# mitchelldurbincs/GeneralsReinforcementLearning

Measured on AMD Instinct MI355X. Metric: env steps/sec (whole node), 20x20 4P fog-on; state bit-exact vs the C restatement of the Go engine (the reference's own test vectors pass on both), higher is better.
Workload: dtype int32

## Files before the change

### generalsreinforcementlearning_amd/csrc/gvec_device.hpp

```cpp
#pragma once
#include <hip/hip_runtime.h>
#include <stdint.h>

#include "../../include/generals_vec.h"

extern "C" __device__ int gvec_llvm_writelane(int value, int lane, int vdst_in) __asm("llvm.amdgcn.writelane.i32");

#ifndef GVEC_NT
#define GVEC_NT 14
#endif
#define GVEC_NT_MASK 2
#define GVEC_NT_PLANE 4
#define GVEC_NT_ARMY 8
#ifndef GVEC_SC1
#define GVEC_SC1 1
#endif

#ifndef GVEC_LEAN
#define GVEC_LEAN 7
#endif

#ifndef GVEC_XLANE
#define GVEC_XLANE 28
#endif
#define GVEC_XL_SPREAD 1
#define GVEC_XL_ROW0 2
#define GVEC_XL_ORROWS 4
#define GVEC_XL_ROWLAST 8
#define GVEC_XL_GATHER 16

namespace gvec {

constexpr bool lean_derive_ok(int nslot) { return (GVEC_LEAN & 1) != 0 && 2 * nslot < 64 / (nslot <= 7 ? 4 : 2); }
constexpr bool lean_half_last(int nslot, bool odd) { return (GVEC_LEAN & 2) != 0 && odd && (nslot & 1) != 0; }
constexpr int lean_fold_dwords(int mutable_planes, int fd) { return (GVEC_LEAN & 4) != 0 ? ((mutable_planes * fd + 3) & ~3) - mutable_planes * fd : 0; }
constexpr bool xlane_tight(int maxp, int nslot) { return maxp >= 8 && nslot <= 1; }
constexpr bool xlane_swaps_ok(int maxp, int nslot) { return !(maxp >= 8 && nslot >= 16) && !xlane_tight(maxp, nslot); }
constexpr bool xlane_spread(int maxp, int nslot) { return (GVEC_XLANE & 1) != 0 && xlane_swaps_ok(maxp, nslot); }
constexpr bool xlane_or_rows(int maxp, int nslot) { return (GVEC_XLANE & 4) != 0 && xlane_swaps_ok(maxp, nslot); }
constexpr bool xlane_gather(int maxp, int nslot) { return (GVEC_XLANE & 16) != 0 && !xlane_tight(maxp, nslot); }

typedef uint32_t u32x4 __attribute__((ext_vector_type(4)));

template <typename T>
__device__ __forceinline__ T ld_stream(const T* p) {
  if constexpr ((GVEC_NT & 1) != 0) return __builtin_nontemporal_load(p);
  return *p;
}
__device__ __forceinline__ void st_through(uint32_t* p, uint32_t v) { asm volatile("global_store_dword %0, %1, off sc1 nt" : : "v"(p), "v"(v) : "memory"); }
__device__ __forceinline__ void st_through(uint16_t* p, uint16_t v) {
  asm volatile("global_store_short %0, %1, off sc1 nt" : : "v"(p), "v"((uint32_t)v) : "memory");
}
__device__ __forceinline__ void st_through(float* p, float v) { asm volatile("global_store_dword %0, %1, off sc1 nt" : : "v"(p), "v"(v) : "memory"); }
__device__ __forceinline__ void st_through(u32x4* p, u32x4 v) {
  asm volatile("global_store_dwordx4 %0, %1, off sc1 nt\n\ts_nop 1" : : "v"(p), "v"(v) : "memory");
}
template <int CLASS, typename T>
__device__ __forceinline__ void st_stream(T* p, T v) {
  if constexpr ((GVEC_NT & CLASS) != 0) {
    if constexpr (GVEC_SC1 != 0) st_through(p, v);
    else __builtin_nontemporal_store(v, p);
  } else {
    *p = v;
  }
}

constexpr int HDR_DW = 24;
enum : int {
  H_TURN = 0,
  H_DIMS = 1,
  H_STATUS = 2,
  H_EPISODE = 3,
  H_ARMYCNT = 4,
  H_GIDX = 12,
  H_RECIPW = 20,
  H_CNT_STEPS = 21,
  H_CNT_ABORT = 22,
  H_CNT_DONE = 23
};
constexpr uint32_t HF_DONE = 1u, HF_FOG = 2u, HF_WIDE = 4u;
constexpr uint32_t HF_SETUP = 8u;
constexpr uint32_t HF_SYNC = 16u;
constexpr uint32_t HF_VSMALL = 32u;
constexpr uint32_t HF_LDIFF = 128u;
constexpr uint32_t HF_FEWSPECIAL = 64u;

template <int MAXP>
struct Planes {
  static constexpr int OWN = 0, VIS = MAXP, CHG = 2 * MAXP, VCH = 2 * MAXP + 1, GT1 = 2 * MAXP + 2,
                       GEN = 2 * MAXP + 3, CITY = 2 * MAXP + 4, MTN = 2 * MAXP + 5, VALID = 2 * MAXP + 6, NCOL0 = 2 * MAXP + 7,
                       NCOLL = 2 * MAXP + 8, OK = 2 * MAXP + 9 , LST = 2 * MAXP + 13,
                       COUNT = 3 * MAXP + 13, MUTABLE = 2 * MAXP + 3, SHARED = 13 ;
};

template <int MAXP_, int NSLOT_, bool ODD_>
struct VariantGeom {
  static constexpr int MAXP = MAXP_, NSLOT = NSLOT_;
  static constexpr bool ODD = ODD_;
  static constexpr int FD = 2 * NSLOT - (ODD ? 1 : 0);
  static constexpr int ROW_DW = (Planes<MAXP>::COUNT * FD + 3) / 4 * 4;
  static constexpr int GYM_STAGE_DW = (NSLOT * 64 * 5 + 15) / 16 * 4;
  static_assert(GYM_STAGE_DW >= NSLOT * 64, "the larger user of the gym step kernels' army shadow: the stage serves as both");
};

constexpr uint32_t KF_AGENT = 1u;
constexpr uint32_t KF_EMIT = 2u;
constexpr uint32_t KF_AUTORESET = 4u;
constexpr uint32_t KF_LMVALID = 16u;

struct StepArgs {
  uint32_t* hdr;
  uint32_t* rows;
  uint32_t* army16;
  int32_t* army32;
  const gvec_action* actions;
  gvec_action* actions_out;
  int32_t* err;
  uint32_t* legal;
  const uint32_t* zeros;
  const uint32_t* pool_hdr;
  const uint32_t* pool_rows;
  const uint32_t* pool_army16;
  const int32_t* pool_army32;
// ... 438 lines not shown
```

### generalsreinforcementlearning_amd/csrc/gvec_kernels.hip

```cpp
#include "gvec_dispatch.hpp"
#include "gvec_turn.hpp"

namespace gvec {

template <int MAXP, int NSLOT>
constexpr int step_waves() {
  const int state = Turn<MAXP, NSLOT>::STATE_REGS;
  return waves_for_regs(state + (state + 32 <= 62 ? 32 : 40));
}

template <int MAXP, int NSLOT, bool AGENT, bool ODD>
__global__ __launch_bounds__(64 * WAVES_PER_BLOCK, (step_waves<MAXP, NSLOT>())) void step_kernel(StepArgs A) {
  constexpr int FD = VariantGeom<MAXP, NSLOT, ODD>::FD, ROW_DW = VariantGeom<MAXP, NSLOT, ODD>::ROW_DW;
  __shared__ int32_t army_shadow[WAVES_PER_BLOCK][NSLOT * 64];
  using B = Turn<MAXP, NSLOT>;
  __shared__ uint32_t act_scratch[WAVES_PER_BLOCK][B::ACT_SCRATCH_DW];
  const int wave = block_wave(), lane = lane_id();
  const int env = wave_item();
  if (env >= A.num_envs) return;
  bool force_redeal = false;
  if constexpr (!AGENT) {
    const uint32_t f0 = (uint32_t)uni((int)reinterpret_cast<const uint32_t*>(A.actions)[((size_t)env * A.pstride) * 2 + 1]);
    if (f0 & GVEC_ACT_SKIP_ENV) {
      if (A.err && lane == 0) A.err[env] = 0;
      return;
    }
    force_redeal = (f0 & GVEC_ACT_RESET_ENV) != 0u;
  }
  B b;
  b.larmy = army_shadow[wave];
  b.lscr = act_scratch[wave];
  const ArmyRef army_env = army_ref<NSLOT>(A.army16, A.army32, env);
  load_turn<true, lean_half_last(NSLOT, ODD)>(b, A.hdr + (size_t)env * HDR_DW, A.rows + (size_t)env * ROW_DW, army_env, FD, A.zeros);
  b.small = !(b.hflags & HF_WIDE);
  const bool emit = (A.flags & KF_EMIT) != 0u;
  uint32_t m[B::NR][4];
  uint32_t err = 0u;
  bool types_dirty = false, changed = true;
  const bool can_redeal = (A.flags & KF_AUTORESET) && A.pool_size > 0;
  if (AGENT && A.actions_out && (b.hflags & HF_DONE)) {
    if (lane < A.pstride) reinterpret_cast<uint2*>(A.actions_out)[(size_t)env * A.pstride + lane] = make_uint2(0u, 0u);
  }
  if (can_redeal && ((b.hflags & HF_DONE) || force_redeal)) {
    redeal<MAXP, NSLOT>(b, A, env, FD, ROW_DW);
    types_dirty = true;
  } else if (b.hflags & HF_DONE) {
    err = GVEC_ERR_GAME_OVER;
    changed = false;
  } else {
    typename B::ActVec av;
    if constexpr (AGENT) {
      b.template legal_planes<false>(m);
      uint32_t mine = (GVEC_PROFILE_SKIP & 1) ? 0u : agent_sample<MAXP, NSLOT>(b, m, env_key_of(A.seed_base, (uint32_t)env), A);
      if (GVEC_PROFILE_DUP & 64) { b.opaque(); b.template legal_planes<false>(m); }
      if (GVEC_PROFILE_DUP & 1) {
        b.opaque();
#pragma unroll
        for (int d = 0; d < 4; ++d) asm volatile("" : "+v"(m[0][d]));
        const uint32_t again = agent_sample<MAXP, NSLOT>(b, m, env_key_of(A.seed_base, (uint32_t)env), A);
        asm volatile("" : : "v"(again));
      }
      av = agent_actvec<MAXP, NSLOT>(b, mine, A.invalid_permille > 0);
      if (A.actions_out) {
        uint32_t alo, ahi;
        agent_words<MAXP, NSLOT>(b, mine, alo, ahi);
        if (lane < A.pstride) reinterpret_cast<uint2*>(A.actions_out)[(size_t)env * A.pstride + lane] = make_uint2(alo, ahi);
      }
    } else {
      uint32_t alo = 0u, ahi = 0u;
      if (lane < A.pstride) {
        const uint2 w = reinterpret_cast<const uint2*>(A.actions)[(size_t)env * A.pstride + lane];
        alo = w.x;
        ahi = w.y;
      }
      av = b.prevalidate(alo, ahi);
    }
    bool aborted;
    err = b.turn_step(av, A, aborted);
    if (!(GVEC_PROFILE_SKIP & 32)) b.refresh_gt1();
    if (GVEC_PROFILE_DUP & 32) { b.opaque_v(); b.refresh_gt1(); }
    hdr_set(b, H_CNT_STEPS, hdr_get(b, H_CNT_STEPS) + 1u);
    if (aborted) hdr_set(b, H_CNT_ABORT, hdr_get(b, H_CNT_ABORT) + 1u);
    if (b.hflags & HF_DONE) hdr_set(b, H_CNT_DONE, hdr_get(b, H_CNT_DONE) + 1u);
  }
  store_army<true>(b, army_env);
  settle_lists(b);
  b.store_hdr(A.hdr + (size_t)env * HDR_DW, err);
  if (types_dirty) b.store_planes(A.rows + (size_t)env * ROW_DW, FD, ROW_DW, true);
  else b.store_planes_staged(A.rows + (size_t)env * ROW_DW, FD);
  if (A.err && lane == 0) A.err[env] = (int32_t)err;
  if (!(GVEC_PROFILE_SKIP & 64) && emit && (changed || !(A.flags & KF_LMVALID))) {
    b.template legal_planes<false>(m);
    b.store_masks_staged(m, A.legal + (size_t)env * A.pstride * A.mask_dw, FD, A.pstride);
  }
}

template <int MAXP, int NSLOT>
__global__ __launch_bounds__(64 * WAVES_PER_BLOCK, (rollout_waves<MAXP, NSLOT>())) void rollout_kernel(StepArgs A) {
  __shared__ int32_t army_shadow[WAVES_PER_BLOCK][NSLOT * 64];
  using B = Turn<MAXP, NSLOT>;
  __shared__ uint32_t act_scratch[WAVES_PER_BLOCK][B::ACT_SCRATCH_DW];
  const int wave = block_wave(), lane = lane_id();
  const int env = wave_item();
  if (env >= A.num_envs) return;
  B b;
  b.larmy = army_shadow[wave];
  b.lscr = act_scratch[wave];
  const ArmyRef army_env = army_ref<NSLOT>(A.army16, A.army32, env);
  load_turn(b, A.hdr + (size_t)env * HDR_DW, A.rows + (size_t)env * A.row_dw, army_env, A.fd, A.zeros);
  uint32_t m[B::NR][4];
  uint32_t err = 0u, n_steps = 0u, n_abort = 0u, n_done = 0u;
  const uint32_t ek = env_key_of(A.seed_base, (uint32_t)env);
  const bool can_redeal = (A.flags & KF_AUTORESET) && A.pool_size > 0;
  int k = 0;
  for (;;) {
    b.template legal_planes<false>(m);
// ... 419 lines not shown
```

### generalsreinforcementlearning_amd/csrc/gvec_packed.hpp

```cpp
#pragma once
#include "gvec_device.hpp"

#ifndef GVEC_PROFILE_SKIP
#define GVEC_PROFILE_SKIP 0
#endif
#ifndef GVEC_PROFILE_DUP
#define GVEC_PROFILE_DUP 0
#endif
#ifndef GVEC_ACT_VECTOR
#define GVEC_ACT_VECTOR 1
#endif

namespace gvec {

template <int ROWL>
__device__ __forceinline__ uint32_t row_scan_add(uint32_t v) {
  v += dpp0<0x111>(v);
  v += dpp0<0x112>(v);
  v += dpp0<0x114>(v);
  v += dpp0<0x118>(v);
  if constexpr (ROWL == 32) v += dpp0<0x142, 0xa>(v);
  return v;
}
template <int ROWL>
// ... 141 lines not shown
  }
  __device__ __forceinline__ void decode_hdr_scalar(const uint32_t* hdr_env) {
    typedef const __attribute__((address_space(4))) uint32_t* kptr;
    unpack_hdr(*this, [k = (kptr)hdr_env](int i) { return k[i]; });
  }
  __device__ __forceinline__ void land_scalars() {
    asm volatile("" : "+s"(turn), "+s"(W), "+s"(H), "+s"(P), "+s"(hflags), "+s"(alive), "+s"(recipW));
  }
  __device__ __forceinline__ void load_hdr(const uint32_t* hdr_env) {
    issue_hdr(hdr_env);
    decode_hdr(*this);
  }
  __device__ __forceinline__ void land() {
    asm volatile("" : "+v"(hv));
#pragma unroll
    for (int k = 0; k < NR; ++k) {
      asm volatile("" : "+v"(own[k]));
      asm volatile("" : "+v"(lst[k]));
      asm volatile("" : "+v"(vis[k]));
    }
#pragma unroll
    for (int k = 0; k < NSR; ++k) asm volatile("" : "+v"(shp[k]));
  }
  __device__ __forceinline__ void opaque() {
    opaque_v();
    asm volatile("" : "+s"(turn), "+s"(alive), "+s"(hflags));
  }
  __device__ __forceinline__ void opaque_v() {
    asm volatile("" : "+v"(hv));
#pragma unroll
    for (int s = 0; s < NSLOT; ++s) asm volatile("" : "+v"(army[s]));
#pragma unroll
    for (int k = 0; k < NR; ++k) {
      asm volatile("" : "+v"(own[k]));
      asm volatile("" : "+v"(lst[k]));
      asm volatile("" : "+v"(vis[k]));
    }
    asm volatile("" : "+v"(chg));
    asm volatile("" : "+v"(vch));
    asm volatile("" : "+v"(gt1));
  }
  __device__ __forceinline__ void store_hdr(uint32_t* hdr_env, uint32_t last_err) { pack_hdr<false, GVEC_NT_PLANE>(*this, hdr_env, last_err); }

  template <bool PACK = true>
  __device__ __forceinline__ void load_planes(const uint32_t* rows_env, int fd, const uint32_t* zeros) {
    const bool in = col() < fd;
    const uint32_t* lane_base = rows_env + (row() * fd + col());
    if constexpr (PACK) {
#pragma unroll
      for (int k = 0; k < NR; ++k) {
        own[k] = vis[k] = 0u;
        if (in && (k * PPR + row() < MAXP)) {
          own[k] = ld_stream(lane_base + (PL::OWN + k * PPR) * fd);
          vis[k] = ld_stream(lane_base + (PL::VIS + k * PPR) * fd);
        }
      }
#pragma unroll
      for (int k = 0; k < NSR; ++k) {
        shp[k] = 0u;
        if (in && (k * PPR + row() < NPACKED)) shp[k] = ld_stream(lane_base + (PL::CHG + k * PPR) * fd);
      }
    } else {
#pragma unroll
      for (int k = 0; k < NR; ++k) {
        const uint32_t* gp = (in && (k * PPR + row() < MAXP)) ? lane_base : zeros;
        own[k] = ld_stream(gp + (PL::OWN + k * PPR) * fd);
        vis[k] = ld_stream(gp + (PL::VIS + k * PPR) * fd);
      }
      load_lists(rows_env, fd);
      const uint32_t* gs = in ? rows_env + col() : zeros;
      chg = ld_stream(gs + PL::CHG * fd);
      vch = ld_stream(gs + PL::VCH * fd);
      gt1 = ld_stream(gs + PL::GT1 * fd);
      gen = ld_stream(gs + PL::GEN * fd);
      city = ld_stream(gs + PL::CITY * fd);
      mtn = ld_stream(gs + PL::MTN * fd);
      valid = ld_stream(gs + PL::VALID * fd);
      ncol0 = ld_stream(gs + PL::NCOL0 * fd);
      ncolL = ld_stream(gs + PL::NCOLL * fd);
#pragma unroll
      for (int d = 0; d < 4; ++d) ok[d] = ld_stream(gs + (PL::OK + d) * fd);
    }
  }
  __device__ __forceinline__ void load_lists(const uint32_t* rows_env, int fd) {
#pragma unroll
    for (int k = 0; k < NR; ++k) lst[k] = own[k];
    if (hflags & HF_LDIFF) {
      const uint32_t* lane_base = rows_env + (row() * fd + col());
#pragma unroll
      for (int k = 0; k < NR; ++k) {
        lst[k] = 0u;
        if (col() < fd && (k * PPR + row() < MAXP)) lst[k] = lane_base[(PL::LST + k * PPR) * fd];
      }
    }
  }
  __device__ __forceinline__ void store_lists(uint32_t* rows_env, int fd) const {
    if (!(hflags & HF_LDIFF)) return;
    uint32_t* gp = rows_env + row() * fd + col();
#pragma unroll
    for (int k = 0; k < NR; ++k)
      if (col() < fd && (k * PPR + row() < MAXP)) gp[(PL::LST + k * PPR) * fd] = lst[k];
  }
  __device__ __forceinline__ uint32_t shared_plane(int j) const {
    return row_to_all<ROWL, XL_SPREAD>(shp[j / PPR], j % PPR);
  }
  __device__ __forceinline__ void spread_shared() {
    chg = shared_plane(PL::CHG - PL::CHG);
    vch = shared_plane(PL::VCH - PL::CHG);
    gt1 = shared_plane(PL::GT1 - PL::CHG);
    gen = shared_plane(PL::GEN - PL::CHG);
    city = shared_plane(PL::CITY - PL::CHG);
    mtn = shared_plane(PL::MTN - PL::CHG);
    valid = shared_plane(PL::VALID - PL::CHG);
    ncol0 = shared_plane(PL::NCOL0 - PL::CHG);
    ncolL = shared_plane(PL::NCOLL - PL::CHG);
    if constexpr (DERIVE_OK) {
      derive_targets(*this);
    } else {
#pragma unroll
      for (int d = 0; d < 4; ++d) ok[d] = shared_plane(PL::OK + d - PL::CHG);
    }
  }
  __device__ __forceinline__ void store_planes(uint32_t* rows_env, int fd, int row_dw, bool with_types) const {
    const bool in = col() < fd;
    uint32_t* gp = rows_env + row() * fd + col();
#pragma unroll
    for (int k = 0; k < NR; ++k) {
      if (in && (k * PPR + row() < MAXP)) {
        st_stream<GVEC_NT_PLANE>(gp + (PL::OWN + k * PPR) * fd, own[k]);
        st_stream<GVEC_NT_PLANE>(gp + (PL::VIS + k * PPR) * fd, vis[k]);
      }
    }
    store_lists(rows_env, fd);
    static_assert(PL::VCH == PL::CHG + 1 && PL::GT1 == PL::CHG + 2, "the three mutable shared planes are stored as rows of one register");
#pragma unroll
    for (int k = 0; k * PPR < 3; ++k) {
      const int j = k * PPR + row();
      if (in && j < 3) st_stream<GVEC_NT_PLANE>(gp + (PL::CHG + k * PPR) * fd, j == 0 ? chg : (j == 1 ? vch : gt1));
    }
    const int lane = lane_id();
    if (lane < fd) {
      uint32_t* g = rows_env + lane;
      if (with_types) {
        g[PL::GEN * fd] = gen;
        g[PL::CITY * fd] = city;
        g[PL::MTN * fd] = mtn;
        g[PL::VALID * fd] = valid;
        g[PL::NCOL0 * fd] = ncol0;
        g[PL::NCOLL * fd] = ncolL;
#pragma unroll
        for (int d = 0; d < 4; ++d) g[(PL::OK + d) * fd] = ok[d];
      }
    }
    if (with_types && lane < row_dw - PL::COUNT * fd) rows_env[PL::COUNT * fd + lane] = 0u;
  }
  template <bool HALF_LAST = false>
  __device__ __forceinline__ void load_army_narrow(const ArmyCRef& a) { army_load_narrow<NSLOT, HALF_LAST>(army, a.n); }
  __device__ __forceinline__ void load_army_wide_if_flagged(const ArmyCRef& a) {
    if (hflags & HF_WIDE) army_load_wide<NSLOT>(army, a.w);
  }

  __device__ __forceinline__ void army_to_lds() {
#pragma unroll
    for (int s = 0; s < NSLOT; ++s) larmy[64 * s + lane_id()] = army[s];
    wave_lds_fence();
  }
  __device__ __forceinline__ void army_from_lds() {
    wave_lds_fence();
#pragma unroll
    for (int s = 0; s < NSLOT; ++s) army[s] = larmy[64 * s + lane_id()];
  }
  static __device__ __forceinline__ void larmy_store(int32_t* p, int32_t v) { *p = v; }
  __device__ __forceinline__ int army_get(int t) const { return uni(larmy[t]); }
  __device__ __forceinline__ void army_set(int t, int val) {
    if (lane_id() == 0) larmy[t] = val;
  }

  __device__ __forceinline__ bool bit_at(uint32_t shared_plane, int t) const { return (rdlane(shared_plane, t >> 5) >> (t & 31)) & 1u; }
  __device__ __forceinline__ bool bit_at_p(const uint32_t (&reg)[NR], int p, int t) const {
    uint32_t w = 0u;
#pragma unroll
    for (int k = 0; k < NR; ++k) {
      const uint32_t r = rdlane(reg[k], player_lane<ROWL>(p, t >> 5));
      w = (k == p / PPR) ? r : w;
    }
    return (w >> (t & 31)) & 1u;
  }
  __device__ __forceinline__ uint32_t tile_bit(int t) const { return (col() == (t >> 5)) ? (1u << (t & 31)) : 0u; }

  static constexpr bool XL_GATHER = xlane_gather(MAXP, NSLOT);
  static __device__ __forceinline__ int32_t gather_mask(uint32_t plane, int s, int row_base = 0) { return gather_mask_as<XL_GATHER>(plane, s, row_base); }
  static __device__ __forceinline__ uint32_t gather(uint32_t plane, int s, int row_base = 0) { return gather_as<XL_GATHER>(plane, s, row_base); }
  static __device__ __forceinline__ uint32_t replicate_row0(uint32_t plane) { return row_to_all<ROWL, (GVEC_XLANE & GVEC_XL_ROW0) != 0>(plane, 0); }
  __device__ __forceinline__ int count_shared(uint32_t plane) const {
    return (int)rdlane(row_scan_add<ROWL>((uint32_t)__builtin_popcount(plane)), ROWL - 1);
  }
  static __device__ __forceinline__ bool any_bit(uint32_t plane) { return __builtin_amdgcn_ballot_w64(plane != 0u) != 0ull; }
  __device__ __forceinline__ void refresh_gt1() {
    uint32_t g = 0u;
#pragma unroll
    for (int s = 0; s < NSLOT; ++s) ballot_to_row0(g, __builtin_amdgcn_ballot_w64(army[s] > 1), s);
    gt1 = replicate_row0(g);
  }

  __device__ __forceinline__ void update_fog(bool matched = false) {
    if (!(hflags & HF_FOG)) return;
    bool full, none;
    if ((hflags & HF_VSMALL) && turn > 0 && P <= N / 10) {
      full = false;
      none = !any_bit(vch);
    } else {
      const int nv = count_shared(vch);
      full = turn == 0 || nv > N / 10;
      none = nv == 0;
    }
    if (full) {
#pragma unroll
      for (int k = 0; k < NR; ++k) {
        const uint32_t d = dil3(lst[k]);
        vis[k] = lane_flag(alive, k) ? d : 0u;
      }
      return;
    }
    if (none) return;
    const uint32_t near3 = dil3(vch), clr = ~near3;
    const uint32_t near5 = matched ? 0u : dil3(near3);
#pragma unroll
    for (int k = 0; k < NR; ++k) {
      const uint32_t d = dil3(lst[k]);
      const unsigned long long hit = __builtin_amdgcn_ballot_w64((matched ? (d & near3) : (own[k] & near5)) != 0u);
      const bool relit = row_slice<ROWL>(hit, row()) != 0u && lane_flag(alive, k);
      vis[k] = (vis[k] & clr) | (relit ? d : 0u);
    }
  }

  __device__ __forceinline__ uint32_t multi_sum(const int32_t (&acc)[MAXP]) const {
    static_assert(MAXP == 2 || MAXP == 4 || MAXP == 8, "fold levels are written for 2, 4 or 8 players");
    static_assert(H_ARMYCNT == 4, "the final row_shl assumes header lanes 4..4+MAXP-1");
    const int lane = lane_id();
    uint32_t m[MAXP];
#pragma unroll
    for (int p = 0; p < MAXP; ++p) m[p] = (uint32_t)acc[p];
    {
      const bool hi = (lane & 1) != 0;
#pragma unroll
      for (int i = 0; i < MAXP / 2; ++i) {
        const uint32_t keep = hi ? m[2 * i + 1] : m[2 * i], give = hi ? m[2 * i] : m[2 * i + 1];
        m[i] = keep + dpp0<0xB1>(give);
      }
    }
    if constexpr (MAXP >= 4) {
      const bool hi = (lane & 2) != 0;
#pragma unroll
      for (int i = 0; i < MAXP / 4; ++i) {
        const uint32_t keep = hi ? m[2 * i + 1] : m[2 * i], give = hi ? m[2 * i] : m[2 * i + 1];
        m[i] = keep + dpp0<0x4E>(give);
      }
    }
    if constexpr (MAXP >= 8) {
      const bool hi = (lane & 4) != 0;
      const uint32_t keep = hi ? m[1] : m[0], give = hi ? m[0] : m[1];
      m[0] = keep + dpp0<0x124>(give);
    }
    uint32_t r = m[0];
    if constexpr (MAXP <= 2) r += dpp0<0x112>(r);
    if constexpr (MAXP <= 4) r += dpp0<0x114>(r);
    r += dpp0<0x118>(r);
    constexpr bool VALU = XL_ORROWS;
    const LanePair h = with_partner<16, VALU>(r);
    r = h.a + h.b;
    const LanePair g = with_partner<32, VALU>(r);
    r = g.a + g.b;
    return dpp0<0x100 + 12 - MAXP>(r);
  }

  __device__ __forceinline__ void update_stats(bool end_of_turn = false, bool delta = false) {
    bool full;
    if (end_of_turn && !grow && (hflags & HF_FEWSPECIAL) && turn > 0) {
      if (!any_bit(chg)) return;
      full = false;
    } else {
      const int nc = count_shared(chg);
      if (nc == 0 && turn > 0) return;
      full = turn == 0 || nc > N / 5;
    }
    uint32_t moved = 0u;
#pragma unroll
    for (int k = 0; k < NR; ++k) {
      const uint32_t nl = full ? own[k] : (own[k] & (lst[k] | chg));
      moved |= nl ^ lst[k];
      lst[k] = nl;
    }
    const int lane = lane_id();
    if (delta && !full && prod_uniform) {
      uint32_t add = dpp0<0x114>((lane < MAXP) ? (uint32_t)move_delta : 0u);
      static_assert(H_ARMYCNT == 4 && MAXP <= 8, "row_shr:4 lands lanes 0..MAXP-1 on the ArmyCount lanes");
      if (prod_rate != 0) {
#pragma unroll
        for (int k = 0; k < NR; ++k) {
          const uint32_t sc = row_scan_add<ROWL>((uint32_t)__builtin_popcount(prod_mask & lst[k]));
          const int p = lane - H_ARMYCNT;
          const uint32_t got = row_result<ROWL>(sc, p & (PPR - 1));
          add += (p >= 0 && p < MAXP && p / PPR == k) ? __umul24(got, (uint32_t)prod_rate) : 0u;
        }
      }
      hv += (lane >= H_ARMYCNT && lane < H_ARMYCNT + MAXP) ? add : 0u;
      hflags |= HF_SYNC;
      if (!any_bit(moved)) return;
    } else {
      int32_t acc[MAXP];
#pragma unroll
      for (int p = 0; p < MAXP; ++p) acc[p] = 0;
      if (small) {
#pragma unroll
        for (int s = 0; s < NSLOT; ++s) {
#pragma unroll
          for (int p = 0; p < MAXP; ++p)
            acc[p] = (int32_t)mad24((uint32_t)army[s], gather(lst[p / PPR], s, player_row<ROWL>(p)), (uint32_t)acc[p]);
        }
      } else {
#pragma unroll
        for (int s = 0; s < NSLOT; ++s) {
#pragma unroll
          for (int p = 0; p < MAXP; ++p) acc[p] += army[s] & gather_mask(lst[p / PPR], s, player_row<ROWL>(p));
        }
      }
      const uint32_t tot = multi_sum(acc);
      hv = (lane >= H_ARMYCNT && lane < H_ARMYCNT + MAXP) ? tot : hv;
      hflags |= HF_SYNC;
    }
    {
      const int hl = lane - H_GIDX;
#pragma unroll
      for (int k = 0; k < NR; ++k) {
        const uint32_t g = lst[k] & gen;
        const int32_t v = row_scan_max<ROWL>((g != 0u) ? (32 * col() + 31 - __builtin_clz(g)) : -1);
        const uint32_t got = row_result<ROWL>((uint32_t)v, hl & (PPR - 1));
        hv = (hl >= 0 && hl < MAXP && hl / PPR == k) ? got : hv;
      }
      alive = (uint32_t)(__builtin_amdgcn_ballot_w64(hl >= 0 && hl < MAXP && (int32_t)hv >= 0) >> H_GIDX) & ((1u << MAXP) - 1u);
    }
  }

  __device__ __forceinline__ void production(int pg, int pc, int pn, int interval, uint32_t interval_magic) {
    if ((uint32_t)turn < 0x10000u && (uint32_t)interval < 0x10000u) {
      const uint32_t q = __umulhi((uint32_t)turn, interval_magic);
      int32_t r = turn - (int32_t)(q * (uint32_t)interval);
      r = r < 0 ? r + interval : r;
      grow = r == 0;
    } else {
      grow = (turn % interval) == 0;
    }
    uint32_t listed_alive = 0u;
#pragma unroll
    for (int k = 0; k < NR; ++k) listed_alive |= lane_flag(alive, k) ? lst[k] : 0u;
    listed_alive = or_rows(listed_alive);
    const uint32_t mg = (pg > 0) ? (listed_alive & gen) : 0u;
    const uint32_t mc = (pc > 0) ? (listed_alive & city) : 0u;
    uint32_t mn = 0u;
    if (grow && pn > 0) mn = listed_alive & ~(gen | city | mtn) & valid;
    chg |= mg | mc | mn;
    const int an = (grow && pn > 0) ? pn : pc;
    prod_uniform = pg == pc && pc == an;
    prod_mask = mg | mc | mn;
    prod_rate = pg;
    if (prod_uniform) {
      const uint32_t m = prod_mask;
#pragma unroll
      for (int s = 0; s < NSLOT; ++s) army[s] = (int32_t)mad24(gather(m, s), (uint32_t)pg, (uint32_t)army[s]);
    } else {
#pragma unroll
      for (int s = 0; s < NSLOT; ++s) army[s] += (pg & gather_mask(mg, s)) + (pc & gather_mask(mc, s)) + (pn & gather_mask(mn, s));
    }
  }

  __device__ __forceinline__ void check_game_over() {
    const int na = __builtin_popcount(alive);
    const int most = (P > 1) ? 1 : 0;
    const bool over = na <= most;
    hflags = over ? (hflags | HF_DONE) : (hflags & ~HF_DONE);
  }

  struct ActVec {
    uint32_t meta;
    int ft, tt;
  };
  __device__ __forceinline__ ActVec prevalidate(uint32_t alo, uint32_t ahi) const {
    ActVec v;
    const int fx = (int)(int8_t)(alo & 0xFFu), fy = (int)(int8_t)((alo >> 8) & 0xFFu);
    const int tx = (int)(int8_t)((alo >> 16) & 0xFFu), ty = (int)(int8_t)(alo >> 24);
    const bool inb = fx >= 0 && fx < W && fy >= 0 && fy < H && tx >= 0 && tx < W && ty >= 0 && ty < H;
    const int dx = fx - tx, dy = fy - ty;
    const int md = (dx < 0 ? -dx : dx) + (dy < 0 ? -dy : dy);
    uint32_t code = 0u;
    code = (md != 1) ? GVEC_ERR_NOT_ADJACENT : code;
    code = (md == 0) ? GVEC_ERR_MOVE_TO_SELF : code;
    code = (!inb) ? GVEC_ERR_INVALID_COORDINATES : code;
    v.meta = code | ((ahi & GVEC_ACT_VALID) ? 16u : 0u) | ((ahi & GVEC_ACT_HALF) ? 32u : 0u);
    v.ft = __mul24(fy, W) + fx;
    v.tt = __mul24(ty, W) + tx;
    return v;
  }

  template <int PID>
  __device__ __forceinline__ void apply_action(const ActVec& av, uint32_t& first_err, uint64_t& orders, int& n_orders,
                                               uint32_t& elim_seen) {
    const uint32_t m = rdlane(av.meta, PID);
    if (!(m & 16u)) return;
    if (!((alive >> PID) & 1u)) return;
    uint32_t code = m & 15u;
    int fa = 0, ta = 0, ft = 0, tt = 0;
    if (!code) {
      ft = (int)rdlane((uint32_t)av.ft, PID);
      tt = (int)rdlane((uint32_t)av.tt, PID);
      fa = army_get(ft);
      ta = army_get(tt);
      if (!bit_at_p(own, PID, ft)) code = GVEC_ERR_NOT_OWNED;
      else if (fa <= 1) code = GVEC_ERR_INSUFFICIENT_ARMY;
      else if (bit_at(mtn, tt)) code = GVEC_ERR_TARGET_IS_MOUNTAIN;
    }
    if (code) {
      first_err = first_err ? first_err : code;
      return;
    }
    int n = (m & 32u) ? (fa / 2) : (fa - 1);
    n = (n == 0) ? 1 : n;
    const uint32_t fbit = tile_bit(ft), tbit = tile_bit(tt);
    army_set(ft, fa - n);
    chg |= fbit | tbit;
    if (bit_at_p(own, PID, tt)) {
      army_set(tt, ta + n);
    } else if (n > ta) {
      int prev = -1;
#pragma unroll
      for (int q = 0; q < MAXP; ++q)
// ... 54 lines not shown
    }
    const bool own_ft = ((w_ft >> (ft & 31)) & 1u) != 0u;
    const bool mine_tt = ((owner_bits >> lane) & 1u) != 0u;
    const bool mtn_tt = ((bperm(tcol << 2, mtn) >> (tt & 31)) & 1u) != 0u;
    const bool gen_tt = ((bperm(tcol << 2, gen) >> (tt & 31)) & 1u) != 0u;
    uint32_t dyn = mtn_tt ? GVEC_ERR_TARGET_IS_MOUNTAIN : 0u;
    dyn = (fa <= 1) ? GVEC_ERR_INSUFFICIENT_ARMY : dyn;
    dyn = own_ft ? dyn : GVEC_ERR_NOT_OWNED;
    const uint32_t code = cand ? dyn : scode;
    const bool ok = cand && dyn == 0u;
    {
      const unsigned long long em = __builtin_amdgcn_ballot_w64(active && code != 0u);
      if (em && !first_err) first_err = rdlane(code, (int)__builtin_ctzll(em));
    }
    int32_t n = (m & 32u) ? (fa >> 1) : (fa - 1);
    n = n < 1 ? 1 : n;
    const bool take = !mine_tt && n > ta;
    const bool capture = ok && take;
    const int32_t fight = take ? n - ta : ta - n;
    const int32_t new_ta = mine_tt ? ta + n : fight;
    larmy_store(ok ? &larmy[ft] : reinterpret_cast<int32_t*>(s_dummy), fa - n);
    larmy_store(ok ? &larmy[tt] : reinterpret_cast<int32_t*>(s_dummy), new_ta);
    atomicOr(ok ? &s_chg[fcol] : s_dummy, fbit);
    atomicOr(ok ? &s_chg[tcol] : s_dummy, tbit);
    atomicOr(capture ? &s_cap[tcol] : s_dummy, tbit);
    atomicOr(capture ? &s_own[64 * (lane / PPR) + myrow + tcol] : s_dummy, tbit);
    const int32_t burnt = take ? ta : n;
    const int32_t loss = (ok && !mine_tt) ? burnt : 0;
    atomicAdd((loss != 0 && owner_bits != 0u) ? &s_loss[__builtin_ctz(owner_bits | 0x80000000u) & 7] : s_dummy, (uint32_t)loss);
    wave_lds_fence();
    move_delta = -(loss + (int32_t)s_loss[lane & 7]);
    const uint32_t capbits = s_cap[col()];
    chg |= s_chg[col()];
    vch |= capbits;
#pragma unroll
    for (int k = 0; k < NR; ++k) own[k] = (own[k] & ~capbits) | s_own[64 * k + lane];
    unsigned long long el = __builtin_amdgcn_ballot_w64(capture && gen_tt);
    if (el) el = __builtin_amdgcn_ballot_w64(capture && gen_tt && owner_bits != 0u);
    while (el) {
      const int p = (int)__builtin_ctzll(el);
      el &= el - 1ull;
      const int prev = (int)__builtin_ctz(rdlane(owner_bits, p));
      if (!((elim_seen >> prev) & 1u)) {
        orders |= (uint64_t)((uint32_t)prev | ((uint32_t)p << 4)) << (8 * n_orders);
        n_orders++;
        elim_seen |= 1u << prev;
      }
    }
    return true;
  }

  template <int PID>
  __device__ __forceinline__ void act_chain(const ActVec& av, uint32_t& first_err, uint64_t& orders, int& n_orders,
                                            uint32_t& elim_seen) {
    if constexpr (PID < MAXP) {
      if (PID < P) apply_action<PID>(av, first_err, orders, n_orders, elim_seen);
      act_chain<PID + 1>(av, first_err, orders, n_orders, elim_seen);
    }
  }

  __device__ __forceinline__ void eliminate(uint64_t orders, int n_orders) {
    for (int e = 0; e < n_orders; ++e) {
      const int v = (int)((orders >> (8 * e)) & 15u), nw = (int)((orders >> (8 * e + 4)) & 15u);
      uint32_t tiles = 0u;
#pragma unroll
      for (int k = 0; k < NR; ++k) tiles |= (lane_player(k) == v) ? (lst[k] & own[k]) : 0u;
      tiles = or_rows(tiles);
#pragma unroll
      for (int k = 0; k < NR; ++k) {
        own[k] = (lane_player(k) == v) ? (own[k] & ~tiles) : own[k];
        own[k] = (lane_player(k) == nw) ? (own[k] | tiles) : own[k];
      }
      hdr_set(*this, H_GIDX + v, 0xFFFFFFFFu);
      chg |= tiles;
      vch |= tiles;
      hflags &= ~HF_VSMALL;
      alive &= ~(1u << v);
    }
  }

  __device__ __forceinline__ uint32_t turn_step(uint32_t acts_lo, uint32_t acts_hi, const StepArgs& A, bool& aborted) {
    return turn_step(prevalidate(acts_lo, acts_hi), A, aborted);
  }
  __device__ __forceinline__ uint32_t turn_step(const ActVec& av, const StepArgs& A, bool& aborted) {
    aborted = false;
    turn++;
    const bool matched = lists_match(*this);
    if (!(GVEC_PROFILE_SKIP & 2)) update_fog(matched);
    if (GVEC_PROFILE_DUP & 2) { opaque(); update_fog(matched); }
    chg = 0u;
    vch = 0u;
    hflags |= HF_VSMALL;
    bool delta = matched && (hflags & HF_SYNC) != 0u;
    move_delta = 0;
    uint32_t first_err = 0u, elim_seen = 0u;
    uint64_t orders = 0ull;
    int n_orders = 0;
    const unsigned long long present = __builtin_amdgcn_ballot_w64((av.meta & 16u) != 0u && lane_id() < P);
    if (present && !(GVEC_PROFILE_SKIP & 4)) {
      army_to_lds();
      if (!(GVEC_ACT_VECTOR && lscr && act_vector(av, first_err, orders, n_orders, elim_seen))) {
        act_chain<0>(av, first_err, orders, n_orders, elim_seen);
        delta = false;
      }
      army_from_lds();
    }
    if (n_orders > 0) {
      eliminate(orders, n_orders);
      update_stats();
    }
    if (first_err) {
      if (n_orders == 0) hflags &= ~HF_SYNC;
      aborted = true;
      return first_err;
    }
    if (!(GVEC_PROFILE_SKIP & 8)) production(A.prod_general, A.prod_city, A.prod_normal, A.interval, A.interval_magic);
    if (!(GVEC_PROFILE_SKIP & 16)) update_stats(n_orders == 0, delta && n_orders == 0);
    if (GVEC_PROFILE_DUP & 16) { opaque_v(); update_stats(n_orders == 0, false); }
    check_game_over();
    return 0u;
  }

  __device__ __forceinline__ void initial_setup() {
    turn = 0;
    chg = 0u;
    vch = 0u;
#pragma unroll
    for (int k = 0; k < NR; ++k) vis[k] = 0u;
    hflags = (hflags & ~HF_DONE) | HF_VSMALL;
    update_stats();
    update_fog();
    check_game_over();
  }

  template <bool SERIALIZER = false>
  __device__ __forceinline__ void legal_planes(uint32_t (&m)[NR][4]) const {
#pragma unroll
    for (int k = 0; k < NR; ++k) {
      const uint32_t s = SERIALIZER ? (own[k] & gt1) : (lst[k] & own[k] & gt1);
      const uint32_t src = (SERIALIZER || lane_flag(alive, k)) ? s : 0u;
      m[k][0] = src & ok[0];
      m[k][1] = src & (SERIALIZER ? ok[2] : ok[1]);
      m[k][2] = src & (SERIALIZER ? ok[3] : ok[2]);
      m[k][3] = src & (SERIALIZER ? ok[1] : ok[3]);
    }
  }
  __device__ __forceinline__ void store_masks(const uint32_t (&m)[NR][4], uint32_t* legal_env, int fd, int pstride) const {
    const bool in = col() < fd;
#pragma unroll
    for (int k = 0; k < NR; ++k) {
      const int p = lane_player(k);
      if (in && p < pstride && p < MAXP) {
        uint32_t* g = legal_env + (size_t)p * (4 * fd) + col();
#pragma unroll
        for (int d = 0; d < 4; ++d) st_stream<GVEC_NT_MASK>(g + d * fd, m[k][d]);
      }
    }
  }
  template <int CLASS>
  __device__ __forceinline__ void flush_stage(uint32_t* dst, int dwords) const {
    const u32x4* s4 = reinterpret_cast<const u32x4*>(larmy);
    u32x4* g4 = reinterpret_cast<u32x4*>(dst);
    const int chunks = dwords >> 2;
    for (int i = lane_id(); i < chunks; i += 64) {
      st_stream<CLASS>(g4 + i, s4[i]);
    }
    const int tail = dwords & 3, l = lane_id();
    if (l < tail) st_stream<CLASS>(dst + 4 * chunks + l, reinterpret_cast<const uint32_t*>(larmy)[4 * chunks + l]);
  }
  __device__ __forceinline__ void store_planes_staged(uint32_t* rows_env, int fd) const {
    uint32_t* stage = reinterpret_cast<uint32_t*>(larmy);
    const bool in = col() < fd;
    uint32_t* g = stage + row() * fd + col();
    wave_lds_fence();
#pragma unroll
    for (int k = 0; k < NR; ++k) {
      if (in && (k * PPR + row() < MAXP)) {
        g[(PL::OWN + k * PPR) * fd] = own[k];
        g[(PL::VIS + k * PPR) * fd] = vis[k];
      }
    }
#pragma unroll
    for (int k = 0; k * PPR < 3; ++k) {
      const int j = k * PPR + row();
      if (in && j < 3) g[(PL::CHG + k * PPR) * fd] = j == 0 ? chg : (j == 1 ? vch : gt1);
    }
    const int gap = lean_fold_dwords(PL::MUTABLE, fd);
    if (in && row() == 0) {
      if (col() < gap) g[PL::GEN * fd] = gen;
      if (fd + col() < gap) g[PL::CITY * fd] = city;
      if (2 * fd + col() < gap) g[PL::MTN * fd] = mtn;
    }
    wave_lds_fence();
    flush_stage<GVEC_NT_PLANE>(rows_env, PL::MUTABLE * fd + gap);
    store_lists(rows_env, fd);
  }
  __device__ __forceinline__ void store_army_narrow_staged(uint32_t* n) const {
    uint32_t* stage = reinterpret_cast<uint32_t*>(larmy);
    const int lane = lane_id();
    wave_lds_fence();
#pragma unroll
// ... 30 lines not shown
```

### generalsreinforcementlearning_amd/csrc/gvec_turn.hpp

```cpp
#pragma once
#include "gvec_launch.hpp"
#include "gvec_packed.hpp"

namespace gvec {

template <int MAXP, int NSLOT>
using Turn = PBoard<MAXP, NSLOT>;

template <int MAXP, int NSLOT>
__device__ __forceinline__ uint32_t agent_sample(const Turn<MAXP, NSLOT>& b, const uint32_t (&m)[Turn<MAXP, NSLOT>::NR][4], uint32_t ek,
                                                 const StepArgs& A) {
  using T = Turn<MAXP, NSLOT>;
  constexpr int NR = T::NR, PPR = T::PPR, ROWL = T::ROWL;
  const int lane = lane_id();
  const uint32_t sbase = ek + (uint32_t)b.turn * 0x9E3779B1u + 0x165667B1u;
  uint32_t mine = 0u;
#pragma unroll
  for (int k = 0; k < NR; ++k) {
    const uint32_t player = (uint32_t)T::lane_player(k);
    const uint32_t h1 = amix(mad24(player, 0x4A7C15u, sbase));
    const uint32_t h2 = amix(h1 ^ 0x68E31DA4u);
    const uint32_t hi16 = h2 >> 16;
    const bool act = b.lane_flag(b.alive, k) && !((h1 & 0xFFFFu) < A.agent_noop);
    const bool half = (h1 >> 16) < A.agent_half;
    const bool inv = A.invalid_permille > 0 && (__umul24(h2 & 0xFFFFu, 1000u) >> 16) < (uint32_t)A.invalid_permille;
    const uint32_t c0 = (uint32_t)__builtin_popcount(m[k][0]), c1 = c0 + (uint32_t)__builtin_popcount(m[k][1]);
    const uint32_t c2 = c1 + (uint32_t)__builtin_popcount(m[k][2]), cnt = c2 + (uint32_t)__builtin_popcount(m[k][3]);
    const uint32_t sc = row_scan_add<ROWL>(cnt);
    const uint32_t total = row_last<ROWL>(sc);
    const uint32_t kk = __umul24(hi16, total) >> 16;
    const uint32_t below = sc - cnt;
    const bool sel = kk >= below && kk < sc;
    const uint32_t r = kk - below;
    const uint32_t d = (r >= c0 ? 1u : 0u) + (r >= c1 ? 1u : 0u) + (r >= c2 ? 1u : 0u);
    const uint32_t base = (d == 0u) ? 0u : (d == 1u) ? c0 : (d == 2u) ? c1 : c2;
    const uint32_t w = (d == 0u) ? m[k][0] : (d == 1u) ? m[k][1] : (d == 2u) ? m[k][2] : m[k][3];
    const uint32_t t_sel = 32u * (uint32_t)T::col() + kth_set_bit(w, r - base);
    const uint32_t pick = row_scan_or<ROWL>(sel ? (t_sel | (d << 10) | 0x8000u) : 0u);
    const uint32_t unchecked = (__umul24(hi16, (uint32_t)b.N) >> 16) | (((h1 >> 8) & 3u) << 10) | 0x8000u;
    const uint32_t fin = inv ? unchecked : pick;
    const bool go = act && (fin & 0x8000u) != 0u;
    const uint32_t out = (fin & 0xFFFu) | (go ? 0x1000u : 0u) | (half ? 0x2000u : 0u);
    const uint32_t got = row_result<ROWL>(out, lane % PPR);
    mine = (lane / PPR == k) ? got : mine;
  }
  return mine;
}

template <int MAXP, int NSLOT>
__device__ __forceinline__ void agent_words(const Turn<MAXP, NSLOT>& b, uint32_t mine, uint32_t& alo, uint32_t& ahi) {
  const bool act = lane_id() < MAXP && (mine & 0x1000u) != 0u;
  const int t = (int)(mine & 0x3FFu), d = (int)((mine >> 10) & 3u);
  const int y = (int)(__umul24((uint32_t)t, (uint32_t)b.recipW) >> 16), x = t - (int)__umul24((uint32_t)y, (uint32_t)b.W);
  const int dx = (d == 1) - (d == 3), dy = (d == 2) - (d == 0);
  const uint32_t lo = ((uint32_t)x & 0xFFu) | (((uint32_t)y & 0xFFu) << 8) | (((uint32_t)(x + dx) & 0xFFu) << 16) |
                      (((uint32_t)(y + dy) & 0xFFu) << 24);
  alo = act ? lo : 0u;
  ahi = act ? (GVEC_ACT_VALID | ((mine & 0x2000u) ? GVEC_ACT_HALF : 0u)) : 0u;
}

template <int MAXP, int NSLOT>
__device__ __forceinline__ typename Turn<MAXP, NSLOT>::ActVec agent_actvec(const Turn<MAXP, NSLOT>& b, uint32_t mine, bool may_be_unchecked) {
  typename Turn<MAXP, NSLOT>::ActVec v;
  const bool act = lane_id() < MAXP && (mine & 0x1000u) != 0u;
  const int t = (int)(mine & 0x3FFu), d = (int)((mine >> 10) & 3u);
  uint32_t code = 0u;
  if (may_be_unchecked) {
    const int y = (int)(__umul24((uint32_t)t, (uint32_t)b.recipW) >> 16), x = t - (int)__umul24((uint32_t)y, (uint32_t)b.W);
    const bool off = (d == 0) ? (y == 0) : (d == 1) ? (x == b.W - 1) : (d == 2) ? (y == b.H - 1) : (x == 0);
    code = off ? GVEC_ERR_INVALID_COORDINATES : 0u;
  }
  v.meta = act ? (code | 16u | ((mine & 0x2000u) ? 32u : 0u)) : 0u;
  v.ft = t;
  v.tt = t + ((d == 0) ? -b.W : (d == 1) ? 1 : (d == 2) ? b.W : -1);
  return v;
}

template <typename BT>
__device__ __forceinline__ void load_board(BT& b, const uint32_t* hdr, const uint32_t* rows, const ArmyCRef& army, int fd) {
  b.load_hdr(hdr);
  load_army(b, army);
  b.load_planes(rows, fd);
}
template <bool EARLY = false, bool HALF_LAST = false, typename BT>
__device__ __forceinline__ void load_turn(BT& b, const uint32_t* hdr, const uint32_t* rows, const ArmyCRef& army, int fd, const uint32_t* zeros) {
  if constexpr (EARLY) {
    b.issue_hdr(hdr);
    b.load_planes(rows, fd, zeros);
    b.template load_army_narrow<HALF_LAST>(army);
    b.decode_hdr_scalar(hdr);
    b.land();
    b.land_scalars();
    b.spread_shared();
    b.load_lists(rows, fd);
    b.load_army_wide_if_flagged(army);
  } else {
    b.load_hdr(hdr);
    load_army(b, army);
    b.template load_planes<false>(rows, fd, zeros);
  }
}

template <int MAXP, int NSLOT, typename BT>
__device__ __forceinline__ void redeal(BT& b, const StepArgs& A, int env, int fd, int row_dw) {
  const uint32_t episode = hdr_get(b, H_EPISODE) + 1u;
  const uint32_t cs = hdr_get(b, H_CNT_STEPS), ca = hdr_get(b, H_CNT_ABORT), cd = hdr_get(b, H_CNT_DONE);
  const uint32_t hk = fmix32(env_key_of(A.pool_seed_base, (uint32_t)env) ^ (episode * 0x9E3779B1u));
  const int j = (int)__umulhi(hk, (uint32_t)A.pool_size);
  load_turn(b, A.pool_hdr + (size_t)j * HDR_DW, A.pool_rows + (size_t)j * row_dw, army_cref<NSLOT>(A.pool_army16, A.pool_army32, j), fd, A.zeros);
  hdr_set(b, H_EPISODE, episode);
  hdr_set(b, H_CNT_STEPS, cs);
  hdr_set(b, H_CNT_ABORT, ca);
  hdr_set(b, H_CNT_DONE, cd);
}

constexpr int waves_for_regs(int need) {
  const int alloc = (need + 7) / 8 * 8;
  const int w = 512 / alloc;
  return w > 8 ? 8 : (w < 2 ? 2 : w);
}
template <int MAXP, int NSLOT>
constexpr int rollout_waves() {
  return waves_for_regs(Turn<MAXP, NSLOT>::STATE_REGS + (NSLOT >= 16 ? 100 : NSLOT >= 10 ? 68 : 44));
}

struct GymView {
  uint32_t own, seen;
};
template <typename B>
__device__ __forceinline__ uint32_t player_view(int pl, const uint32_t (&reg)[B::NR]) {
  uint32_t out = 0u;
#pragma unroll
  for (int k = 0; k < B::NR; ++k) {
    const uint32_t g = bperm(player_lane<B::ROWL>(pl, B::col()) << 2, reg[k]);
    out = (pl / B::PPR == k) ? g : out;
  }
  return out;
}
template <typename B>
__device__ __forceinline__ GymView turn_view(const B& b, int pl) {
  const uint32_t own_p = player_view<B>(pl, b.own);
  return GymView{own_p, (b.hflags & HF_FOG) ? player_view<B>(pl, b.vis) : b.valid};
}
template <typename BT>
__device__ __forceinline__ uint32_t gym_sources(const BT& b, const GymView& v) {
  return v.own & v.seen & b.gt1;
}

template <typename B>
__device__ __forceinline__ uint32_t turn_tile_counts(const B& b) {
  const int lane = lane_id();
  uint32_t tcl = 0u;
#pragma unroll
  for (int k = 0; k < B::NR; ++k) {
    const uint32_t sc = row_scan_add<B::ROWL>((uint32_t)__builtin_popcount(b.lst[k]));
    const uint32_t got = row_result<B::ROWL>(sc, lane % B::PPR);
    tcl = (lane / B::PPR == k) ? got : tcl;
  }
  return tcl;
}
template <int MAXP, typename BT>
__device__ __forceinline__ uint32_t army_counts(const BT& b) {
  return bperm((H_ARMYCNT + (lane_id() & (MAXP - 1))) << 2, b.hv);
}

__device__ __forceinline__ int gym_winner(bool over, int P, uint32_t alive) {
// ... 39 lines not shown
```

Before: 1.256 billion.

## Add specialized fast path for ordinary non-growth turns in step kernel

Adds a compile-time specialized step path, used when the header flags show a synced, small, few-special, non-wide, non-done env with no growth on the coming turn. On that path the list diff load, wide army load, list-match check and growth computation are skipped, and the fog/stats updates take their delta branches unconditionally. Header/planes/army loads are split into an issue phase and a tail so the ordinary-turn decision is made before the rest is loaded. This trades extra code size and register pressure for less branching and fewer loads on the common turn, and it relies on the flag predicates exactly matching the conditions the general path checks.

```diff
diff --git a/generalsreinforcementlearning_amd/csrc/gvec_device.hpp b/generalsreinforcementlearning_amd/csrc/gvec_device.hpp
--- a/generalsreinforcementlearning_amd/csrc/gvec_device.hpp
+++ b/generalsreinforcementlearning_amd/csrc/gvec_device.hpp
@@ -29,6 +29,12 @@
 #define GVEC_XL_ROWLAST 8
 #define GVEC_XL_GATHER 16
 
+#ifndef GVEC_ORDTURN
+#define GVEC_ORDTURN 5
+#endif
+#define GVEC_OT_PATH 1
+#define GVEC_OT_NOGROW 4
+
 namespace gvec {
 
 constexpr bool lean_derive_ok(int nslot) { return (GVEC_LEAN & 1) != 0 && 2 * nslot < 64 / (nslot <= 7 ? 4 : 2); }
@@ -39,6 +45,13 @@
 constexpr bool xlane_spread(int maxp, int nslot) { return (GVEC_XLANE & 1) != 0 && xlane_swaps_ok(maxp, nslot); }
 constexpr bool xlane_or_rows(int maxp, int nslot) { return (GVEC_XLANE & 4) != 0 && xlane_swaps_ok(maxp, nslot); }
 constexpr bool xlane_gather(int maxp, int nslot) { return (GVEC_XLANE & 16) != 0 && !xlane_tight(maxp, nslot); }
+constexpr bool ordturn_fits(int maxp, int nslot, bool agent, bool odd) {
+  if (!agent) return maxp <= 4 ? nslot <= 7 : nslot <= 1;
+  return maxp <= 2 || (maxp <= 4 ? nslot <= 10 : (nslot <= 2 && !(nslot == 2 && odd)));
+}
+constexpr int ordturn_bits(int maxp, int nslot, bool agent, bool odd) {
+  return (GVEC_ORDTURN & GVEC_OT_PATH) != 0 && ordturn_fits(maxp, nslot, agent, odd) ? (GVEC_ORDTURN & (GVEC_OT_PATH | GVEC_OT_NOGROW)) : 0;
+}
 
 typedef uint32_t u32x4 __attribute__((ext_vector_type(4)));
 
diff --git a/generalsreinforcementlearning_amd/csrc/gvec_kernels.hip b/generalsreinforcementlearning_amd/csrc/gvec_kernels.hip
--- a/generalsreinforcementlearning_amd/csrc/gvec_kernels.hip
+++ b/generalsreinforcementlearning_amd/csrc/gvec_kernels.hip
@@ -7,6 +7,50 @@
 constexpr int step_waves() {
   const int state = Turn<MAXP, NSLOT>::STATE_REGS;
   return waves_for_regs(state + (state + 32 <= 62 ? 32 : 40));
+}
+
+template <int ORD, int MAXP, int NSLOT, bool AGENT, bool ODD>
+__device__ __forceinline__ void step_ordinary(Turn<MAXP, NSLOT>& b, const StepArgs& A, int env, const uint32_t* rows_in, const ArmyRef& army_env) {
+  constexpr int FD = VariantGeom<MAXP, NSLOT, ODD>::FD, ROW_DW = VariantGeom<MAXP, NSLOT, ODD>::ROW_DW;
+  using B = Turn<MAXP, NSLOT>;
+  const int lane = lane_id();
+  load_turn_tail<ORD>(b, rows_in, army_env, FD);
+  b.small = true;
+  uint32_t m[B::NR][4];
+  typename B::ActVec av;
+  if constexpr (AGENT) {
+    b.template legal_planes<false>(m);
+    const uint32_t mine = agent_sample<MAXP, NSLOT>(b, m, env_key_of(A.seed_base, (uint32_t)env), A);
+    av = agent_actvec<MAXP, NSLOT>(b, mine, A.invalid_permille > 0);
+    if (A.actions_out) {
+      uint32_t alo, ahi;
+      agent_words<MAXP, NSLOT>(b, mine, alo, ahi);
+      if (lane < A.pstride) reinterpret_cast<uint2*>(A.actions_out)[(size_t)env * A.pstride + lane] = make_uint2(alo, ahi);
+    }
+  } else {
+    uint32_t alo = 0u, ahi = 0u;
+    if (lane < A.pstride) {
+      const uint2 w = reinterpret_cast<const uint2*>(A.actions)[(size_t)env * A.pstride + lane];
+      alo = w.x;
+      ahi = w.y;
+    }
+    av = b.prevalidate(alo, ahi);
+  }
+  bool aborted;
+  const uint32_t err = b.template turn_step<ORD>(av, A, aborted);
+  b.refresh_gt1();
+  hdr_set(b, H_CNT_STEPS, hdr_get(b, H_CNT_STEPS) + 1u);
+  if (aborted) hdr_set(b, H_CNT_ABORT, hdr_get(b, H_CNT_ABORT) + 1u);
+  if (b.hflags & HF_DONE) hdr_set(b, H_CNT_DONE, hdr_get(b, H_CNT_DONE) + 1u);
+  store_army<true>(b, army_env);
+  settle_lists(b);
+  b.store_hdr(A.hdr + (size_t)env * HDR_DW, err);
+  b.store_planes_staged(A.rows + (size_t)env * ROW_DW, FD);
+  if (A.err && lane == 0) A.err[env] = (int32_t)err;
+  if (A.flags & KF_EMIT) {
+    b.template legal_planes<false>(m);
+    b.store_masks_staged(m, A.legal + (size_t)env * A.pstride * A.mask_dw, FD, A.pstride);
+  }
 }
 
 template <int MAXP, int NSLOT, bool AGENT, bool ODD>
@@ -31,7 +75,18 @@
   b.larmy = army_shadow[wave];
   b.lscr = act_scratch[wave];
   const ArmyRef army_env = army_ref<NSLOT>(A.army16, A.army32, env);
-  load_turn<true, lean_half_last(NSLOT, ODD)>(b, A.hdr + (size_t)env * HDR_DW, A.rows + (size_t)env * ROW_DW, army_env, FD, A.zeros);
+  constexpr int ORD = (GVEC_PROFILE_SKIP | GVEC_PROFILE_DUP) != 0 ? 0 : ordturn_bits(MAXP, NSLOT, AGENT, ODD);
+  if constexpr (ORD != 0) {
+    const uint32_t* rows_env = A.rows + (size_t)env * ROW_DW;
+    load_turn_issue<lean_half_last(NSLOT, ODD)>(b, A.hdr + (size_t)env * HDR_DW, rows_env, army_env, FD, A.zeros);
+    if (!force_redeal && b.template ordinary_turn<ORD>(A)) {
+      step_ordinary<ORD, MAXP, NSLOT, AGENT, ODD>(b, A, env, rows_env, army_env);
+      return;
+    }
+    load_turn_tail<0>(b, rows_env, army_env, FD);
+  } else {
+    load_turn<true, lean_half_last(NSLOT, ODD)>(b, A.hdr + (size_t)env * HDR_DW, A.rows + (size_t)env * ROW_DW, army_env, FD, A.zeros);
+  }
   b.small = !(b.hflags & HF_WIDE);
   const bool emit = (A.flags & KF_EMIT) != 0u;
   uint32_t m[B::NR][4];
diff --git a/generalsreinforcementlearning_amd/csrc/gvec_packed.hpp b/generalsreinforcementlearning_amd/csrc/gvec_packed.hpp
--- a/generalsreinforcementlearning_amd/csrc/gvec_packed.hpp
+++ b/generalsreinforcementlearning_amd/csrc/gvec_packed.hpp
@@ -247,10 +247,11 @@
       for (int d = 0; d < 4; ++d) ok[d] = ld_stream(gs + (PL::OK + d) * fd);
     }
   }
+  template <int ORD = 0>
   __device__ __forceinline__ void load_lists(const uint32_t* rows_env, int fd) {
 #pragma unroll
     for (int k = 0; k < NR; ++k) lst[k] = own[k];
-    if (hflags & HF_LDIFF) {
+    if (!ORD && (hflags & HF_LDIFF)) {
       const uint32_t* lane_base = rows_env + (row() * fd + col());
 #pragma unroll
       for (int k = 0; k < NR; ++k) {
@@ -266,6 +267,26 @@
     for (int k = 0; k < NR; ++k)
       if (col() < fd && (k * PPR + row() < MAXP)) gp[(PL::LST + k * PPR) * fd] = lst[k];
   }
+  static __device__ __forceinline__ bool growth_turn(int t, int interval, uint32_t interval_magic) {
+    bool g;
+    if ((uint32_t)t < 0x10000u && (uint32_t)interval < 0x10000u) {
+      const uint32_t q = __umulhi((uint32_t)t, interval_magic);
+      int32_t r = t - (int32_t)(q * (uint32_t)interval);
+      r = r < 0 ? r + interval : r;
+      g = r == 0;
+    } else {
+      g = (t % interval) == 0;
+    }
+    return g;
+  }
+  template <int ORD>
+  __device__ __forceinline__ bool ordinary_turn(const StepArgs& A) const {
+    constexpr uint32_t need = HF_SYNC | HF_VSMALL | HF_FEWSPECIAL, bar = HF_DONE | HF_WIDE | HF_LDIFF;
+    bool ord = (hflags & (need | bar)) == need && turn >= 0 && 10 * P <= N;
+    if constexpr ((ORD & GVEC_OT_NOGROW) != 0) ord = ord && !growth_turn(turn + 1, A.interval, A.interval_magic);
+    return ord;
+  }
+
   __device__ __forceinline__ uint32_t shared_plane(int j) const {
     return row_to_all<ROWL, XL_SPREAD>(shp[j / PPR], j % PPR);
   }
@@ -321,8 +342,9 @@
   }
   template <bool HALF_LAST = false>
   __device__ __forceinline__ void load_army_narrow(const ArmyCRef& a) { army_load_narrow<NSLOT, HALF_LAST>(army, a.n); }
+  template <int ORD = 0>
   __device__ __forceinline__ void load_army_wide_if_flagged(const ArmyCRef& a) {
-    if (hflags & HF_WIDE) army_load_wide<NSLOT>(army, a.w);
+    if (!ORD && (hflags & HF_WIDE)) army_load_wide<NSLOT>(army, a.w);
   }
 
   __device__ __forceinline__ void army_to_lds() {
@@ -368,10 +390,11 @@
     gt1 = replicate_row0(g);
   }
 
+  template <int ORD = 0>
   __device__ __forceinline__ void update_fog(bool matched = false) {
     if (!(hflags & HF_FOG)) return;
     bool full, none;
-    if ((hflags & HF_VSMALL) && turn > 0 && P <= N / 10) {
+    if (ORD || ((hflags & HF_VSMALL) && turn > 0 && P <= N / 10)) {
       full = false;
       none = !any_bit(vch);
     } else {
@@ -439,15 +462,16 @@
     return dpp0<0x100 + 12 - MAXP>(r);
   }
 
+  template <int ORD = 0>
   __device__ __forceinline__ void update_stats(bool end_of_turn = false, bool delta = false) {
     bool full;
-    if (end_of_turn && !grow && (hflags & HF_FEWSPECIAL) && turn > 0) {
+    if (end_of_turn && !grow && (ORD || ((hflags & HF_FEWSPECIAL) && turn > 0))) {
       if (!any_bit(chg)) return;
       full = false;
     } else {
       const int nc = count_shared(chg);
-      if (nc == 0 && turn > 0) return;
-      full = turn == 0 || nc > N / 5;
+      if (nc == 0 && (ORD || turn > 0)) return;
+      full = (!ORD && turn == 0) || nc > N / 5;
     }
     uint32_t moved = 0u;
 #pragma unroll
@@ -476,7 +500,7 @@
       int32_t acc[MAXP];
 #pragma unroll
       for (int p = 0; p < MAXP; ++p) acc[p] = 0;
-      if (small) {
+      if (ORD || small) {
 #pragma unroll
         for (int s = 0; s < NSLOT; ++s) {
 #pragma unroll
@@ -507,15 +531,10 @@
     }
   }
 
+  template <int ORD = 0>
   __device__ __forceinline__ void production(int pg, int pc, int pn, int interval, uint32_t interval_magic) {
-    if ((uint32_t)turn < 0x10000u && (uint32_t)interval < 0x10000u) {
-      const uint32_t q = __umulhi((uint32_t)turn, interval_magic);
-      int32_t r = turn - (int32_t)(q * (uint32_t)interval);
-      r = r < 0 ? r + interval : r;
-      grow = r == 0;
-    } else {
-      grow = (turn % interval) == 0;
-    }
+    if constexpr ((ORD & GVEC_OT_NOGROW) != 0) grow = false;
+    else grow = growth_turn(turn, interval, interval_magic);
     uint32_t listed_alive = 0u;
 #pragma unroll
     for (int k = 0; k < NR; ++k) listed_alive |= lane_flag(alive, k) ? lst[k] : 0u;
@@ -736,16 +755,17 @@
   __device__ __forceinline__ uint32_t turn_step(uint32_t acts_lo, uint32_t acts_hi, const StepArgs& A, bool& aborted) {
     return turn_step(prevalidate(acts_lo, acts_hi), A, aborted);
   }
+  template <int ORD = 0>
   __device__ __forceinline__ uint32_t turn_step(const ActVec& av, const StepArgs& A, bool& aborted) {
     aborted = false;
     turn++;
-    const bool matched = lists_match(*this);
-    if (!(GVEC_PROFILE_SKIP & 2)) update_fog(matched);
-    if (GVEC_PROFILE_DUP & 2) { opaque(); update_fog(matched); }
+    const bool matched = ORD ? true : lists_match(*this);
+    if (!(GVEC_PROFILE_SKIP & 2)) update_fog<ORD>(matched);
+    if (GVEC_PROFILE_DUP & 2) { opaque(); update_fog<ORD>(matched); }
     chg = 0u;
     vch = 0u;
     hflags |= HF_VSMALL;
-    bool delta = matched && (hflags & HF_SYNC) != 0u;
+    bool delta = ORD ? true : matched && (hflags & HF_SYNC) != 0u;
     move_delta = 0;
     uint32_t first_err = 0u, elim_seen = 0u;
     uint64_t orders = 0ull;
@@ -761,16 +781,16 @@
     }
     if (n_orders > 0) {
       eliminate(orders, n_orders);
-      update_stats();
+      update_stats<ORD>();
     }
     if (first_err) {
       if (n_orders == 0) hflags &= ~HF_SYNC;
       aborted = true;
       return first_err;
     }
-    if (!(GVEC_PROFILE_SKIP & 8)) production(A.prod_general, A.prod_city, A.prod_normal, A.interval, A.interval_magic);
-    if (!(GVEC_PROFILE_SKIP & 16)) update_stats(n_orders == 0, delta && n_orders == 0);
-    if (GVEC_PROFILE_DUP & 16) { opaque_v(); update_stats(n_orders == 0, false); }
+    if (!(GVEC_PROFILE_SKIP & 8)) production<ORD>(A.prod_general, A.prod_city, A.prod_normal, A.interval, A.interval_magic);
+    if (!(GVEC_PROFILE_SKIP & 16)) update_stats<ORD>(n_orders == 0, delta && n_orders == 0);
+    if (GVEC_PROFILE_DUP & 16) { opaque_v(); update_stats<ORD>(n_orders == 0, false); }
     check_game_over();
     return 0u;
   }
diff --git a/generalsreinforcementlearning_amd/csrc/gvec_turn.hpp b/generalsreinforcementlearning_amd/csrc/gvec_turn.hpp
--- a/generalsreinforcementlearning_amd/csrc/gvec_turn.hpp
+++ b/generalsreinforcementlearning_amd/csrc/gvec_turn.hpp
@@ -82,6 +82,21 @@
   load_army(b, army);
   b.load_planes(rows, fd);
 }
+template <bool HALF_LAST, typename BT>
+__device__ __forceinline__ void load_turn_issue(BT& b, const uint32_t* hdr, const uint32_t* rows, const ArmyCRef& army, int fd, const uint32_t* zeros) {
+  b.issue_hdr(hdr);
+  b.load_planes(rows, fd, zeros);
+  b.template load_army_narrow<HALF_LAST>(army);
+  b.decode_hdr_scalar(hdr);
+  b.land();
+  b.land_scalars();
+}
+template <int ORD, typename BT>
+__device__ __forceinline__ void load_turn_tail(BT& b, const uint32_t* rows, const ArmyCRef& army, int fd) {
+  b.spread_shared();
+  b.template load_lists<ORD>(rows, fd);
+  b.template load_army_wide_if_flagged<ORD>(army);
+}
 template <bool EARLY = false, bool HALF_LAST = false, typename BT>
 __device__ __forceinline__ void load_turn(BT& b, const uint32_t* hdr, const uint32_t* rows, const ArmyCRef& army, int fd, const uint32_t* zeros) {
   if constexpr (EARLY) {
```

After: 1.309 billion (median of 6 runs). 4.2% higher.
